# re-ovo/wgpu-path-tracing

Measured on AMD Instinct MI355X. Metric: Msamples/s (rays x bounces / s), higher is better.
Workload: dtype f32

## Files before the change

include/ptmi.h:

```cpp
#ifndef PTMI_H
#define PTMI_H

#include <stddef.h>
#include <stdint.h>
#include "ptmi_layout.h"

#ifdef __cplusplus
extern "C" {
#endif

#define PTMI_ABI_VERSION 4

enum {
    PTMI_OK = 0,
    PTMI_E_INVALID = -1,
    PTMI_E_NODEVICE = -2,
    PTMI_E_HIP = -3,
    PTMI_E_STATE = -4,
    PTMI_E_UNSUPPORTED = -5
};

enum { PTMI_ATLAS_RGBA16F = 1, PTMI_ATLAS_RGBA32F = 2 };
enum { PTMI_TRAVERSAL_AUTO = 0, PTMI_TRAVERSAL_GLOBAL = 1, PTMI_TRAVERSAL_LDS = 2, PTMI_TRAVERSAL_GLOBAL_EXACT = 3 };

// ... 16 lines not shown
    uint32_t tree_builder;
    uint32_t leaves;
    uint32_t leaf_tris;
    uint32_t reserved[1];
} ptmi_options;

typedef struct ptmi_stats {
    uint64_t paths;
    uint64_t segments;
    uint64_t shadow_rays;
    uint64_t dispatches;
    uint64_t frames;
    uint64_t segments_by_bounce[64];
    double   gpu_ms;
    double   extend_ms;
    uint64_t extend_launches;
    double   shade_ms;
    double   shadow_ms;
    uint32_t bvh_depth;
    uint32_t traversal_used;
    uint32_t frames_per_batch_used;
    uint32_t radiance_stride_bytes;
    uint64_t shadow_traced;
    uint64_t shade_launches, shadow_launches;
    double   raygen_ms, compact_ms, accumulate_ms;
    double   upload_ms;
    double   upload_tree_ms;
    double   upload_copy_ms;
    uint32_t leaves_used;
    uint32_t leaf_tris_used;
    uint32_t extend_variant, shadow_variant;
    uint64_t verify_failed;
    uint32_t tree_builder_used;
    uint32_t reserved_stats[1];
} ptmi_stats;

int ptmi_abi_version(void);
int ptmi_create(int device_ordinal, ptmi_ctx **out);
int ptmi_destroy(ptmi_ctx *ctx);
const char *ptmi_last_error(const ptmi_ctx *ctx);

int ptmi_upload_scene(ptmi_ctx *ctx,
                      const ptmi_triangle *triangles, uint32_t n_triangles,
                      const ptmi_material *materials, uint32_t n_materials,
                      const ptmi_bvh_node *bvh_nodes, uint32_t n_nodes,
                      const ptmi_light *lights, uint32_t n_lights);
int ptmi_upload_atlas(ptmi_ctx *ctx, const void *texels, uint32_t width, uint32_t height, int format);
int ptmi_resize(ptmi_ctx *ctx, uint32_t width, uint32_t height);
int ptmi_set_options(ptmi_ctx *ctx, const ptmi_options *opt);
int ptmi_get_options(const ptmi_ctx *ctx, ptmi_options *opt);

int ptmi_dispatch(ptmi_ctx *ctx, const ptmi_camera *camera, uint32_t n_frames);
int ptmi_synchronize(ptmi_ctx *ctx);
int ptmi_throttle(ptmi_ctx *ctx, uint32_t max_in_flight, uint32_t *in_flight);

int ptmi_read_output(ptmi_ctx *ctx, float *dst_rgba, size_t n_floats);
int ptmi_write_output(ptmi_ctx *ctx, const float *src_rgba, size_t n_floats);
void *ptmi_output_device_ptr(ptmi_ctx *ctx);
int ptmi_bind_output_device(ptmi_ctx *ctx, void *device_ptr, size_t bytes);
int ptmi_set_stream(ptmi_ctx *ctx, void *hip_stream);

enum { PTMI_AOV_ALBEDO = 1u, PTMI_AOV_NORMAL = 2u, PTMI_AOV_ID = 4u };
int ptmi_set_aovs(ptmi_ctx *ctx, uint32_t mask);
int ptmi_get_aovs(const ptmi_ctx *ctx, uint32_t *mask);
int ptmi_read_aov(ptmi_ctx *ctx, uint32_t which, void *dst, size_t n_bytes);
void *ptmi_aov_device_ptr(ptmi_ctx *ctx, uint32_t which);

// ... 99 lines not shown
```

wgpu-path-tracing_amd/csrc/pt_device.h:

```cpp
#pragma once
#include <hip/hip_runtime.h>
#include <stdint.h>
#include "ptmi_layout.h"
#include "ptmi.h"

#define PT_HD __host__ __device__ inline

#define PT_REF_LEAF      0x80000000u
#define PT_REF_NONE      0xFFFFFFFFu
#define PT_LEAF_MAX_TRIS 32u
#define PT_LEAF_OFF_BITS 26u
#define PT_LEAF_OFF_MASK ((1u << PT_LEAF_OFF_BITS) - 1u)

struct DevScene;
struct DevScene {
    const ptmi_triangle *tris;  uint32_t n_tris;
    const ptmi_material *mats;  uint32_t n_mats;
    const ptmi_light *lights;   uint32_t n_lights;
    const void *atlas;          uint32_t atlas_w, atlas_h, atlas_fmt;
    const float4 *wnodes;       uint32_t n_wnodes;
    const float4 *tripos;
    float root_min[3], root_max[3];
    uint32_t root_ref;
    const float4 *ref_wnodes;   uint32_t ref_root_ref, has_fast;
    const uint4 *qnodes;        const uint32_t *leaf_stream;
    float q_origin[3], q_scale[3];
    float tri_safe_dsum;
    uint32_t q_cached;
    uint32_t own, n_own_tris;
    const float4 *ref_tripos;
    const float4 *tri_leafbox;
    float ref_root_min[3], ref_root_max[3];
    float safe_origin;
    const float4 *wnodes16, *ref_wnodes16;
    uint32_t root_ref16, ref_root_ref16;
    const uint4 *qnodes16;
    unsigned long long *verify_stat;
    const DevScene *self;
};

struct rgb_sc { float x, y, z; };
struct DevPaths {
    float4 *O, *D; float2 *C; float *L; uint32_t l_stride = 3;
    __device__ __forceinline__ rgb_sc ldL(uint32_t p) const {
        if (l_stride == 4u) { const float4 v = reinterpret_cast<const float4 *>(L)[p]; return rgb_sc{v.x, v.y, v.z}; }
        return reinterpret_cast<const rgb_sc *>(L)[p];
    }
    __device__ __forceinline__ void stL(uint32_t p, float x, float y, float z) const {
        if (l_stride == 4u) reinterpret_cast<float4 *>(L)[p] = make_float4(x, y, z, 0.0f);
        else reinterpret_cast<rgb_sc *>(L)[p] = rgb_sc{x, y, z};
    }
};
struct DevShadow { float4 *SO, *SD; rgb_sc *SC; uint32_t cap; };

struct DevBand {
    uint32_t width, height, y0, y1, strip, parts, part, rows;
    PT_HD uint32_t row_of(uint32_t l) const {
        if (parts <= 1u) return y0 + l;
        return y0 + ((l / strip) * parts + part) * strip + l % strip;
    }
    PT_HD size_t frame_pixel(uint32_t pix) const { return (size_t)row_of(pix / width) * width + pix % width; }
};

PT_HD bool pt_plays_roulette(uint32_t bounce) { return bounce > 2u; }
inline uint32_t pt_repack_bounce() { uint32_t b = 0; while (!pt_plays_roulette(b)) b++; return b; }

struct ShadeParams {
    uint32_t bounce, max_bounces, do_mis;
    unsigned long long *stats;
    uint32_t emit_records;
    const uint32_t *pid;
};
// ... 141 lines not shown
```

wgpu-path-tracing_amd/csrc/ptmi_api.hip:

```cpp
#include "ptmi.h"
#include "pt_device.h"
#include "fast_tree.h"

#include <algorithm>
#include <chrono>
#include <cmath>
#include <cstdarg>
#include <cstdint>
#include <cstdio>
#include <cstring>
#include <deque>
#include <memory>
#include <string>
#include <typeinfo>
#include <utility>
#include <vector>

namespace {

thread_local std::string g_create_err;

enum SceneBuf {
    kTris, kMats, kLights,
    kRefWnodes, kRefTripos,
    kWnodes, kTripos,
    kQnodes, kLeafStream,
    kLeafbox,
    kWnodes16, kRefWnodes16, kQnodes16,
    kSceneBufs
};

enum FramePlane {
    kOut,
    kAovAlbedo, kAovNormal, kAovId,
    kMoments,
    kDnGuide, kDnGrad, kDnA, kDnB, kDnOut,
    kAdBallot, kAdList, kAdTileSums,
    kBlitF32, kBlitU8,
    kFramePlanes
};

enum LaneBuf {
    kPathO, kPathD, kPathC, kPathL,
    kHits,
    kShadow0, kShadowIdx0, kShadow1, kShadowIdx1,
    kTailO, kTailD, kTailC, kPid,
    kQueue0, kQueue1,
    kOcc,
    kAovRec,
    kLaneBufs
};

struct EventPair { hipEvent_t a, b; int kind; };
constexpr size_t kMaxPendingEvents = 4096;

}

struct Lane {
    size_t cap = 0;
    void *buf[kLaneBufs] = {};
    DevPaths paths{};
// ... 744 lines not shown

int ptmi_destroy(ptmi_ctx *c) {
    if (!c) return PTMI_E_INVALID;
    (void)hipSetDevice(c->device);
    (void)sync_all(c);
    drain_events(c);
    for (hipEvent_t e : c->in_flight) (void)hipEventDestroy(e);
    for (hipEvent_t e : c->event_pool) (void)hipEventDestroy(e);
    {
        Lane &ln = c->lane;
        free_batch(ln);
        dfree(ln.counts); dfree(ln.d_spill); dfree(ln.d_spill_side);
        for (hipEvent_t e : {ln.ev_ready, ln.ev_shadow[0], ln.ev_shadow[1]}) if (e) (void)hipEventDestroy(e);
        if (ln.side) (void)hipStreamDestroy(ln.side);
    }
    for (void *&p : c->buf) dfree(p);
    dfree(c->d_atlas);
    drop_planes(c, kAllPlanes);
    dfree(c->d_stats); dfree(c->d_scene); dfree(c->ad.ctl); dfree(c->ad.acc);
    if (c->own_stream) (void)hipStreamDestroy(c->own_stream);
    delete c;
    return PTMI_OK;
}

}

struct PtPrepared {
    Built b;
    uint32_t nt, nm, nl;
    double build_ms;
    bool take_device_buffers = false;
};

PtPrepared *pt_prepare_scene(ptmi_ctx *c, const ptmi_triangle *tris, uint32_t nt, const ptmi_material *mats, uint32_t nm,
                             const ptmi_bvh_node *nodes, uint32_t nn, const ptmi_light *lights, uint32_t nl, int *rc_out) {
    auto bad = [&](int rc) -> PtPrepared * { *rc_out = rc; return nullptr; };
    if (!c) return bad(PTMI_E_INVALID);
    if ((nt && !tris) || (nm && !mats) || (nn && !nodes) || (nl && !lights))
        return bad(fail(c, PTMI_E_INVALID, "NULL blob with a non-zero count"));
    if (hipSetDevice(c->device) != hipSuccess) return bad(fail(c, PTMI_E_HIP, "hipSetDevice(%d) failed", c->device));
    for (uint32_t i = 0; i < nl; i++) {
        if (lights[i].light_type > PTMI_LIGHT_POINT)
            return bad(fail(c, PTMI_E_INVALID, "light %u has unknown type %u", i, lights[i].light_type));
        if (lights[i].light_type == PTMI_LIGHT_EMISSIVE && lights[i].triangle_index >= nt)
            return bad(fail(c, PTMI_E_INVALID, "emissive light %u references triangle %u of %u", i, lights[i].triangle_index, nt));
    }
    const auto t_start = std::chrono::steady_clock::now();
    PtPrepared *p = new PtPrepared();
    int rc = build_image(c->opt, c->stream, c->device, tris, nt, nodes, nn, p->b, c->err);
    if (rc) { delete p; return bad(rc); }
    if (!p->b.buf[kTris].present) p->b.view(kTris, tris, (size_t)nt * sizeof(ptmi_triangle));
    p->b.view(kMats, mats, (size_t)nm * sizeof(ptmi_material));
    p->b.view(kLights, lights, (size_t)nl * sizeof(ptmi_light));
    p->nt = nt; p->nm = nm; p->nl = nl;
    p->build_ms = std::chrono::duration<double, std::milli>(std::chrono::steady_clock::now() - t_start).count();
    *rc_out = PTMI_OK;
    return p;
}
void pt_free_prepared(PtPrepared *p) { delete p; }

int pt_install_scene(ptmi_ctx *c, PtPrepared *prep) {
    if (!c || !prep) return PTMI_E_INVALID;
    HIP_TRY(c, hipSetDevice(c->device));
    using clk = std::chrono::steady_clock;
    auto ms_since = [](clk::time_point t0) { return std::chrono::duration<double, std::milli>(clk::now() - t0).count(); };
    const auto t_start = clk::now();
    Built &b = prep->b;
    const auto t_copy = clk::now();
    void *n[kSceneBufs] = {};
    hipError_t e = hipSuccess;
    for (int k = 0; k < kSceneBufs && e == hipSuccess; k++) {
        HeldBuf &h = b.buf[k];
        if (!h.present) continue;
        if (h.dev && prep->take_device_buffers && h.device == c->device) { n[k] = h.dev; h.dev = nullptr; continue; }
        e = hipMalloc(&n[k], h.bytes ? h.bytes : 16);
        if (e != hipSuccess) break;
        if (h.dev) e = h.device == c->device ? hipMemcpy(n[k], h.dev, h.bytes, hipMemcpyDeviceToDevice)
                                             : hipMemcpyPeer(n[k], c->device, h.dev, h.device, h.bytes);
        else e = h.bytes ? hipMemcpy(n[k], h.host, h.bytes, hipMemcpyHostToDevice) : hipMemset(n[k], 0, 16);
    }
    if (e != hipSuccess) {
        for (void *&p : n) dfree(p);
        return fail(c, PTMI_E_HIP, "scene upload failed: %s (the previous scene, if any, is still in place)", hipGetErrorString(e));
    }
    HIP_TRY(c, sync_all(c));
    for (int k = 0; k < kSceneBufs; k++) { dfree(c->buf[k]); c->buf[k] = n[k]; }
    void *const *d = c->buf;
    const ptmi_image_info &h = b.img;
    const bool own = h.leaves_used == 2u;
    DevScene &s = c->sc;
    s.tris = static_cast<const ptmi_triangle *>(d[kTris]); s.n_tris = prep->nt;
    s.mats = static_cast<const ptmi_material *>(d[kMats]); s.n_mats = prep->nm;
    s.lights = static_cast<const ptmi_light *>(d[kLights]); s.n_lights = prep->nl;
    s.ref_wnodes = static_cast<const float4 *>(d[kRefWnodes]); s.ref_root_ref = b.ref_root_ref; s.has_fast = d[kWnodes] ? 1u : 0u;
    s.wnodes = static_cast<const float4 *>(walked(d, kWnodes));
    s.n_wnodes = h.n_wnodes;
    s.tripos = static_cast<const float4 *>(walked(d, kTripos));
    s.ref_tripos = static_cast<const float4 *>(d[kRefTripos]);
    s.qnodes = static_cast<const uint4 *>(d[kQnodes]); s.leaf_stream = static_cast<const uint32_t *>(d[kLeafStream]);
    for (int k = 0; k < 3; k++) { s.q_origin[k] = h.q_origin[k]; s.q_scale[k] = h.q_scale[k]; }
    s.q_cached = b.q_top;
    s.tri_safe_dsum = b.tri_safe_dsum;
    for (int k = 0; k < 3; k++) {
        s.ref_root_min[k] = b.ref_root_min[k]; s.ref_root_max[k] = b.ref_root_max[k];
        s.root_min[k] = h.root_min[k]; s.root_max[k] = h.root_max[k];
    }
    s.root_ref = h.root_ref;
    s.own = own ? 1u : 0u;
    s.n_own_tris = own ? h.n_tris : 0u;
    s.tri_leafbox = static_cast<const float4 *>(d[kLeafbox]);
    s.wnodes16 = static_cast<const float4 *>(d[kWnodes16]); s.ref_wnodes16 = static_cast<const float4 *>(d[kRefWnodes16]);
    s.qnodes16 = static_cast<const uint4 *>(d[kQnodes16]);
    s.root_ref16 = b.root_ref16; s.ref_root_ref16 = b.ref_root_ref16;
    s.safe_origin = h.safe_origin;
    s.verify_stat = c->d_stats + 4;
    s.self = c->d_scene;
    HIP_TRY(c, hipMemcpy(c->d_scene, &c->sc, sizeof(DevScene), hipMemcpyHostToDevice));
    c->img = h;
    c->have_scene = true;
    c->st.leaves_used = h.leaves_used;
    c->st.leaf_tris_used = h.max_leaf_tris;
    c->st.tree_builder_used = b.tree_builder_used;
    c->st.upload_copy_ms = ms_since(t_copy);
    c->st.upload_tree_ms = b.tree_ms;
    c->st.upload_ms = prep->build_ms + ms_since(t_start);
    return PTMI_OK;
}

extern "C" {

int ptmi_upload_scene(ptmi_ctx *c, const ptmi_triangle *tris, uint32_t nt, const ptmi_material *mats, uint32_t nm,
                      const ptmi_bvh_node *nodes, uint32_t nn, const ptmi_light *lights, uint32_t nl) {
    int rc = PTMI_OK;
    PtPrepared *p = pt_prepare_scene(c, tris, nt, mats, nm, nodes, nn, lights, nl, &rc);
    if (!p) return rc;
    p->take_device_buffers = true;
    rc = pt_install_scene(c, p);
    pt_free_prepared(p);
    return rc;
}

}

int pt_atlas_bytes(uint32_t w, uint32_t h, int fmt, size_t *bytes, char *why, size_t why_len) {
    *bytes = 0;
    if (fmt != PTMI_ATLAS_RGBA16F && fmt != PTMI_ATLAS_RGBA32F) {
        snprintf(why, why_len, "unknown atlas format %d", fmt);
        return PTMI_E_INVALID;
    }
// ... 100 lines not shown
    const uint64_t npix = (uint64_t)band.rows * band.width;
    uint32_t F = c->opt.frames_per_batch;
    const bool auto_F = F == 0;
    Lane &ln = c->lane;
    if (auto_F) {
        F = (uint32_t)std::max<uint64_t>(1, std::min<uint64_t>(64, (128ull << 20) / npix));
        size_t free_b = 0, total_b = 0;
        if (hipMemGetInfo(&free_b, &total_b) == hipSuccess) {
            const uint64_t held = (uint64_t)ln.cap * bytes_per_path(ln.aov != nullptr);
            const uint64_t room = (uint64_t)((double)(free_b + held) * 0.9);
            F = (uint32_t)std::max<uint64_t>(1, std::min<uint64_t>(F, room / (npix * bytes_per_path(c->aov_mask != 0))));
        }
    }
    F = std::min(F, n_frames);
    const bool nee = c->opt.do_mis && c->sc.n_lights > 0;
    const bool side = nee && c->opt.overlap != 0;
    if (npix * F > 0xFFFFFF00ull) return fail(c, PTMI_E_UNSUPPORTED, "batch of %llu paths exceeds 2^32", (unsigned long long)(npix * F));
    const TraverseConfig cfg0 = traverse_config(c, true), cfg_shadow0 = traverse_config(c, false);
    if (c->opt.traversal == PTMI_TRAVERSAL_LDS && pt_variant(cfg0.variant).where != PT_LDS_ALL)
        return fail(c, PTMI_E_UNSUPPORTED, "scene needs %zu B of LDS plus the stack; it does not fit in %zu B", lds_scene_bytes(c), kLdsMax);
    for (;;) {
        rc = ensure_capacity(c, ln, (size_t)(npix * F));
        if (rc == PTMI_OK) break;
        if (!auto_F || !c->alloc_oom || F <= 1) return rc;
        F = (F + 1) / 2;
    }
    if (cfg0.wants_spill && !ln.d_spill) HIP_TRY(c, hipMalloc(&ln.d_spill, pt_spill_bytes(c->n_cu * 8)));
    if (cfg_shadow0.wants_spill && !ln.d_spill_side) HIP_TRY(c, hipMalloc(&ln.d_spill_side, pt_spill_bytes(c->n_cu * 8)));
    c->st.traversal_used = pt_variant(cfg0.variant).where == PT_FROM_MEMORY ? PTMI_TRAVERSAL_GLOBAL : PTMI_TRAVERSAL_LDS;
    c->st.extend_variant = pt_variant_code(cfg0);
    c->st.shadow_variant = pt_variant_code(cfg_shadow0);
    c->st.frames_per_batch_used = F;
    c->st.radiance_stride_bytes = (walks_memory_quantised(cfg0) || walks_memory_quantised(cfg_shadow0)) ? 16u : 12u;
    const int blocks = c->n_cu * 8;
#ifndef PT_SHADE_WGS_PER_CU
#define PT_SHADE_WGS_PER_CU 16
#endif
    const int shade_blocks = c->n_cu * PT_SHADE_WGS_PER_CU;
    const uint32_t maxb = c->opt.max_bounces;
    const bool t1 = c->opt.timing >= 1, t2 = c->opt.timing >= 2, t3 = c->opt.timing >= 3;
    {
        Timed td(c, 0, t1);
        const hipStream_t ms = c->stream;
        const hipStream_t ss = side ? ln.side : ms;
        const int tiles = (int)(ln.cap / pt_compact_tile_slots() + 1);
        TraverseConfig cfg = cfg0, cfg_shadow = cfg_shadow0;
        cfg.spill = ln.d_spill; cfg_shadow.spill = side ? ln.d_spill_side : ln.d_spill;
        if (cfg_shadow.wants_spill && !cfg_shadow.spill) cfg_shadow.spill = ln.d_spill_side;
        ln.paths.l_stride = c->st.radiance_stride_bytes / 4u;
        const DevPaths bp = ln.paths;
        const uint32_t rb = PT_REPACK ? pt_repack_bounce() : 0xFFFFFFFEu;
        DevPaths tp = ln.tail;
        tp.L = bp.L; tp.l_stride = bp.l_stride;
        float4 *const aov_rec = c->aov_mask ? ln.aov : nullptr;
        float4 *const mom = plane_as<float4>(c, kMoments);
        if (ap && cam->frame_index == 0u) { pt_launch_adaptive_restart(ms, blocks, band, mom); c->ad_rounds = 0; }
        auto batch = [&](uint32_t frame0, uint32_t fb) -> int {
            const DevPixels px = ap ? DevPixels{band, 0u, c->ad.list, &c->ad.ctl[1], mom, c->ad.acc}
                                    : DevPixels{band, frame0, nullptr, nullptr, nullptr, nullptr};
            { Timed t(c, 4, t3, ms); pt_launch_raygen(ms, blocks, *cam, px, fb, bp, &ln.counts[0]); }
            int cur = 0;
            for (uint32_t b = 0; b < maxb; b++) {
                const bool tail = b > rb;
                const uint32_t *q = b == 0 || b == rb + 1 ? nullptr : ln.queue[cur];
                const DevPaths sp = tail ? tp : bp;
                const int par = side ? (int)(b & 1u) : 0;
// ... 572 lines not shown
```

wgpu-path-tracing_amd/csrc/shade.hip:

```cpp
#include "pt_device.h"
#include "pt_math.h"

namespace {

struct HitInfo {
    v3 position; float t;
    v3 normal;
    v3 albedo;
    float roughness, metallic, transmission, ior;
    v3 emission; float emissive_strength;
    bool is_front;
};

PT_DEV v3 ld3(const float *p) { return mk3(p[0], p[1], p[2]); }

PT_DEV v4 atlas_load(const DevScene &sc, uint32_t x, uint32_t y) {
    v4 r; r.x = r.y = r.z = r.w = 0.0f;
    if (sc.atlas_fmt == 0u || x >= sc.atlas_w || y >= sc.atlas_h) return r;
    size_t idx = ((size_t)y * sc.atlas_w + x);
    if (sc.atlas_fmt == 1u) {
        const uint2 raw = reinterpret_cast<const uint2 *>(sc.atlas)[idx];
        union { uint32_t u; _Float16 h[2]; } a, b;
        a.u = raw.x; b.u = raw.y;
        r.x = (float)a.h[0]; r.y = (float)a.h[1]; r.z = (float)b.h[0]; r.w = (float)b.h[1];
    } else {
        const float4 t = reinterpret_cast<const float4 *>(sc.atlas)[idx];
        r.x = t.x; r.y = t.y; r.z = t.z; r.w = t.w;
    }
    return r;
}

PT_DEV v4 texture_color(const DevScene &sc, const ptmi_atlas_rect &tx, float uvx, float uvy, v4 fallback) {
    if (tx.w == 0u || tx.h == 0u) return fallback;
    float fx = uvx - __builtin_truncf(uvx);
    float fy = uvy - __builtin_truncf(uvy);
    float ax = (float)tx.x + fx * (float)tx.w;
    float ay = (float)tx.y + fy * (float)tx.h;
    return atlas_load(sc, f2u(ax), f2u(ay));
}

PT_DEV HitInfo make_hitinfo(const DevScene &sc, v3 ro, v3 rd, float t, uint32_t tri) {
    HitInfo hi;
    const ptmi_triangle &T = sc.tris[tri];
    const v3 tv0 = ld3(T.v0), tv1 = ld3(T.v1), tv2 = ld3(T.v2);
    const v3 tn0 = ld3(T.n0), tn1 = ld3(T.n1), tn2 = ld3(T.n2);
    const float u0x = T.uv0[0], u0y = T.uv0[1], u1x = T.uv1[0], u1y = T.uv1[1], u2x = T.uv2[0], u2y = T.uv2[1];
    const uint32_t mi = T.material_index;
    v3 v0 = tv0;
    v3 e1 = sub3(tv1, v0), e2 = sub3(tv2, v0);
    float u, v;
    (void)tri_test(v0, e1, e2, ro, rd, u, v);
    hi.t = t;
    hi.position = madd3(rd, t, ro);
    float w = 1.0f - u - v;
    v3 geo_n = normalize3(cross3(e1, e2));
    v3 n_i = normalize3(lincomb3(tn0, w, tn1, u, tn2, v));
    float uvx = fma1(u2x, v, fma1(u1x, u, u0x * w));
    float uvy = fma1(u2y, v, fma1(u1y, u, u0y * w));
    hi.is_front = dot3(geo_n, rd) < 0.0f;
    ptmi_material m;
    if (mi < sc.n_mats) m = sc.mats[mi];
    else __builtin_memset(&m, 0, sizeof m);
    v4 one; one.x = one.y = one.z = one.w = 1.0f;
    v4 alb = texture_color(sc, m.albedo_map, uvx, uvy, one);
    hi.albedo = mk3(alb.x * m.base_color[0], alb.y * m.base_color[1], alb.z * m.base_color[2]);
    v4 pbr = texture_color(sc, m.pbr_map, uvx, uvy, one);
    hi.metallic = pbr.z * m.metallic;
    hi.roughness = max1(pbr.y * m.roughness, 0.04f);
    hi.transmission = m.transmission;
    hi.ior = m.ior;
    v4 em = texture_color(sc, m.emissive_map, uvx, uvy, one);
    hi.emission = mk3(em.x * m.emission[0], em.y * m.emission[1], em.z * m.emission[2]);
    hi.emissive_strength = m.emissive_strength;
    v4 flat; flat.x = 0.5f; flat.y = 0.5f; flat.z = 1.0f; flat.w = 1.0f;
    v4 nm = texture_color(sc, m.normal_map, uvx, uvy, flat);
    if (nm.x != 0.5f || nm.y != 0.5f || nm.z != 1.0f) {
        float du1x = u1x - u0x, du1y = u1y - u0y;
        float du2x = u2x - u0x, du2y = u2y - u0y;
        float rr = rcp1(fma1(du1x, du2y, -(du1y * du2x)));
        v3 tg = mk3(fma1(e1.x, du2y, -(e2.x * du1y)) * rr, fma1(e1.y, du2y, -(e2.y * du1y)) * rr,
                    fma1(e1.z, du2y, -(e2.z * du1y)) * rr);
        tg = normalize3(tg);
        v3 N = n_i;
        v3 Tn = normalize3(madd3(N, -dot3(N, tg), tg));
        v3 Bn = normalize3(cross3(N, Tn));
        float tx = nm.x * 2.0f - 1.0f, ty = nm.y * 2.0f - 1.0f, tz = nm.z * 2.0f - 1.0f;
        hi.normal = normalize3(lincomb3(Tn, tx, Bn, ty, N, tz));
    } else {
        hi.normal = n_i;
    }
    return hi;
}

PT_DEV float distribution_ggx(v3 N, v3 H, float roughness) {
    float a = roughness * roughness;
// ... 72 lines not shown
    float ndh = max1(dot3(normal, H), 0.0f);
    float vdh = max1(dot3(V, H), 0.0f);
    v3 F0 = mk3(mix1(0.04f, h.albedo.x, h.metallic), mix1(0.04f, h.albedo.y, h.metallic),
                mix1(0.04f, h.albedo.z, h.metallic));
    v3 F = fresnel_schlick(vdh, F0);
    float G = geometry_smith(normal, V, L, h.roughness);
    float D = distribution_ggx(normal, H, h.roughness);
    float one_m_tr = 1.0f - h.transmission;
    v3 kD = mk3((1.0f - F.x) * one_m_tr, (1.0f - F.y) * one_m_tr, (1.0f - F.z) * one_m_tr);
    v3 diffuse = vdiv3(mul3(kD, h.albedo), PT_PI);
    v3 specular = vdiv3(scale3(scale3(F, G), D), max1(4.0f * ndv * ndl, PT_EPS));
    v3 bsdf = mk3(0.0f, 0.0f, 0.0f);
    float pdf = 0.0f;
    if (h.transmission > 0.0f) {
        float eta = front ? rcp1(h.ior) : h.ior;
        float cos_t = dot3(normal, V);
        float Ft = reflectance(__builtin_fabsf(cos_t), eta);
        bsdf = scale3(h.albedo, 1.0f - Ft);
        pdf = (1.0f - h.metallic) * h.transmission;
    } else {
        bsdf = scale3(add3(diffuse, specular), ndl);
        float diffuse_p = (1.0f - h.metallic) * (1.0f - h.transmission);
        float specular_p = h.metallic;
        float diffuse_pdf = ndl / PT_PI;
        float specular_pdf = D * ndh / (4.0f * vdh);
        pdf = diffuse_p * diffuse_pdf + specular_p * specular_pdf;
    }
    v4 r; r.x = bsdf.x; r.y = bsdf.y; r.z = bsdf.z; r.w = max1(pdf, PT_EPS);
    return r;
}

struct LightSample { v3 intensity; v3 wi; float pdf; float dist; bool traced; };

PT_DEV LightSample sample_light(const DevScene &sc, uint32_t &rng, v3 hit_pos) {
    LightSample ls;
    ls.intensity = mk3(0.0f, 0.0f, 0.0f); ls.wi = mk3(0.0f, 0.0f, 0.0f); ls.pdf = 0.0f; ls.dist = -1.0f; ls.traced = false;
    const uint32_t nl = sc.n_lights;
    const ptmi_light lt = sc.lights[rng_int(rng, 0u, nl - 1u)];
    const float inv_n = rcp1((float)nl);
    if (lt.light_type == PTMI_LIGHT_DIRECTIONAL) {
        ls.wi = normalize3(neg3(ld3(lt.position)));
        ls.intensity = scale3(ld3(lt.color), lt.intensity);
        ls.pdf = inv_n * 1000.0f;
        ls.dist = -1.0f;
        ls.traced = true;
    } else if (lt.light_type == PTMI_LIGHT_POINT) {
        v3 to_l = sub3(ld3(lt.position), hit_pos);
        float dist = length3(to_l);
        if (dist > 100.0f) return ls;
        ls.wi = vdiv3(to_l, dist);
        float att = rcp1(dist * dist);
        ls.intensity = scale3(scale3(ld3(lt.color), lt.intensity), att);
        ls.pdf = inv_n * 10000.0f;
        ls.dist = dist;
        ls.traced = true;
    } else if (lt.light_type == PTMI_LIGHT_EMISSIVE) {
        ptmi_triangle T;
        if (lt.triangle_index < sc.n_tris) T = sc.tris[lt.triangle_index];
        else __builtin_memset(&T, 0, sizeof T);
        float r1 = rng_f(rng), r2 = rng_f(rng);
        float sq = sqrt1(r1);
        float u = 1.0f - sq;
        float v = r2 * sq;
        float w = 1.0f - u - v;
        v3 lp = lincomb3(ld3(T.v0), w, ld3(T.v1), u, ld3(T.v2), v);
        v3 n = normalize3(lincomb3(ld3(T.n0), w, ld3(T.n1), u, ld3(T.n2), v));
        v3 to_l = sub3(lp, hit_pos);
        float dist = length3(to_l);
        v3 wi = vdiv3(to_l, dist);
        v3 e1 = sub3(ld3(T.v1), ld3(T.v0)), e2 = sub3(ld3(T.v2), ld3(T.v0));
        float area = length3(cross3(e1, e2)) * 0.5f;
        float cos_t = __builtin_fabsf(dot3(n, neg3(wi)));
        ls.pdf = (inv_n * rcp1(area)) * (dist * dist / max1(cos_t, PT_EPS));
        ls.intensity = scale3(ld3(lt.color), lt.intensity);
        ls.wi = wi;
        ls.dist = dist;
        ls.traced = true;
    }
    return ls;
}

constexpr int SBLOCK = 256;
#ifndef PT_SHADE_WAVES
#define PT_SHADE_WAVES 0
#endif
#if PT_SHADE_WAVES > 0
#define PT_SHADE_ATTR __attribute__((amdgpu_waves_per_eu(PT_SHADE_WAVES)))
#else
#define PT_SHADE_ATTR
#endif

template <bool AOV>
__global__ __launch_bounds__(SBLOCK) PT_SHADE_ATTR void k_shade(DevScene sc, DevPaths P, const uint32_t *__restrict__ queue,
                                                  const uint32_t *__restrict__ count_ptr,
                                                  const float2 *__restrict__ hits, DevShadow S,
                                                  uint64_t *__restrict__ alive_mask,
                                                  uint64_t *__restrict__ shadow_mask, ShadeParams sp,
                                                  float4 *__restrict__ aov) {
    const uint32_t count = *count_ptr;
    const uint32_t lane = threadIdx.x & 63u;
    uint32_t n_skipped = 0, n_emitted = 0;
    for (uint32_t base = blockIdx.x * SBLOCK; base < count; base += gridDim.x * SBLOCK) {
        const uint32_t i = base + threadIdx.x;
        bool alive = false, shadow = false, skipped = false, emitted = false;
        float4 rec_o = make_float4(0.0f, 0.0f, 0.0f, -2.0f), rec_d = make_float4(0.0f, 0.0f, 0.0f, 0.0f);
        rgb_sc rec_c{0.0f, 0.0f, 0.0f};
        if (i < count) {
            const uint32_t q = queue ? queue[i] : i;
            const float2 h2 = ld_stream(&hits[i]);
            if (!(h2.x < 0.0f)) {
                const float4 o4 = ld_stream(&P.O[q]), d4 = ld_stream(&P.D[q]);
                const uint32_t p = sp.pid ? sp.pid[q] : q;
                uint32_t rng = __float_as_uint(o4.w);
                const v3 ro = xyz(o4), rd = xyz(d4);
                v3 thr = mk3(1.0f, 1.0f, 1.0f);
                if (sp.bounce != 0u) { const float2 c2 = ld_stream(&P.C[q]); thr = mk3(d4.w, c2.x, c2.y); }
                const HitInfo hit = make_hitinfo(sc, ro, rd, h2.x, __float_as_uint(h2.y));
                if (AOV) {
                    st_stream(&aov[2 * (size_t)i], make_float4(hit.albedo.x, hit.albedo.y, hit.albedo.z, hit.t));
                    st_stream(&aov[2 * (size_t)i + 1], make_float4(hit.normal.x, hit.normal.y, hit.normal.z, h2.y));
                }
                if (hit.emission.x > 0.0f || hit.emission.y > 0.0f || hit.emission.z > 0.0f) {
                    float att = rcp1(1.0f + hit.t * hit.t);
                    float k = hit.emissive_strength;
                    const v3 e = mk3(thr.x * hit.emission.x * k * att, thr.y * hit.emission.y * k * att, thr.z * hit.emission.z * k * att);
                    if (sp.emit_records) {
                        rec_d.w = __uint_as_float(p);
                        rec_c = rgb_sc{e.x, e.y, e.z};
                        shadow = true; emitted = true;
                    } else {
                        const rgb_sc l = P.ldL(p);
                        P.stL(p, l.x + e.x, l.y + e.y, l.z + e.z);
                    }
                } else {
                    if (sp.do_mis && sc.n_lights > 0u && hit.transmission == 0.0f && hit.is_front) {
                        LightSample ls = sample_light(sc, rng, hit.position);
                        if (ls.pdf > 0.0f) {
                            v3 V = neg3(normalize3(rd));
                            v4 ev = eval_bsdf(hit, hit.normal, V, ls.wi, hit.is_front);
                            float wmis = power_heuristic(1.0f, ls.pdf, 1.0f, ev.w);
                            v3 direct = vdiv3(scale3(mul3(ls.intensity, mk3(ev.x, ev.y, ev.z)), wmis),
                                              max1(ls.pdf, PT_EPS));
                            v3 contrib = mul3(thr, direct);
                            if ((contrib.x != 0.0f) | (contrib.y != 0.0f) | (contrib.z != 0.0f)) {
                                v3 so = madd3(ls.wi, PT_EPS, hit.position);
                                rec_o = make_float4(so.x, so.y, so.z, ls.dist);
                                rec_d = make_float4(ls.wi.x, ls.wi.y, ls.wi.z, __uint_as_float(p));
                                rec_c = rgb_sc{contrib.x, contrib.y, contrib.z};
                                shadow = true;
                            } else {
                                skipped = true;
                            }
                        } else if (ls.traced) {
                            skipped = true;
                        }
                    }
                    v3 dir = sample_bsdf(rng, hit, rd, hit.is_front);
                    v4 ev = eval_bsdf(hit, hit.normal, neg3(normalize3(rd)), dir, hit.is_front);
                    if (!(ev.w <= 0.0f)) {
                        v3 no = madd3(dir, PT_EPS, hit.position);
                        v3 nd = normalize3(dir);
                        thr = mul3(thr, vdiv3(mk3(ev.x, ev.y, ev.z), max1(ev.w, PT_EPS)));
                        alive = true;
                        if (pt_plays_roulette(sp.bounce)) {
                            float pr = max1(max1(thr.x, thr.y), thr.z);
                            if (rng_f(rng) > pr) alive = false;
                            else thr = vdiv3(thr, pr);
                        }
                        if (alive && sp.bounce + 1u < sp.max_bounces) {
// ... 18 lines not shown
                        shadow = true; emitted = true;
                    } else {
                        const rgb_sc l = P.ldL(p);
                        P.stL(p, l.x + e.x, l.y + e.y, l.z + e.z);
                    }
                }
            }
        }
        const uint64_t am = __ballot(alive), sm = __ballot(shadow), zm = __ballot(skipped), em = __ballot(emitted);
        if (shadow) {
            const uint32_t r = (i & ~63u) + (uint32_t)__popcll(sm & ((1ull << lane) - 1ull));
            st_stream(&S.SO[r], rec_o);
            st_stream(&S.SD[r], rec_d);
            S.SC[r] = rec_c;
        }
        if (lane == 0u && i < count) {
            alive_mask[i >> 6] = am;
            shadow_mask[i >> 6] = sm;
            n_skipped += (uint32_t)__popcll(zm);
            n_emitted += (uint32_t)__popcll(em);
        }
    }
    if (n_skipped) atomicAdd(&sp.stats[1], (unsigned long long)n_skipped);
    if (n_emitted) atomicAdd(&sp.stats[3], (unsigned long long)n_emitted);
}

}

#ifdef PT_SHADE_FAST
#define PT_LAUNCH_SHADE pt_launch_shade_fast
#else
#define PT_LAUNCH_SHADE pt_launch_shade
#endif
void PT_LAUNCH_SHADE(hipStream_t s, int blocks, const DevScene &sc, DevPaths p, const uint32_t *queue,
                     const uint32_t *count, const float2 *hits, DevShadow sh, uint64_t *alive_mask,
                     uint64_t *shadow_mask, ShadeParams sp, float4 *aov) {
    if (aov)
        hipLaunchKernelGGL(k_shade<true>, dim3(blocks), dim3(SBLOCK), 0, s, sc, p, queue, count, hits, sh, alive_mask,
                           shadow_mask, sp, aov);
    else
        hipLaunchKernelGGL(k_shade<false>, dim3(blocks), dim3(SBLOCK), 0, s, sc, p, queue, count, hits, sh, alive_mask,
                           shadow_mask, sp, aov);
}

#ifndef PT_SHADE_FAST
namespace {
__global__ void k_hit_uv(uint32_t n, DevScene sc, DevPaths P, const float2 *__restrict__ hits, float2 *__restrict__ uv) {
    const uint32_t i = blockIdx.x * blockDim.x + threadIdx.x;
    if (i >= n) return;
    const float2 h = hits[i];
    float u = 0.0f, v = 0.0f;
    if (!(h.x < 0.0f)) {
        const ptmi_triangle &T = sc.tris[__float_as_uint(h.y)];
        const v3 v0 = ld3(T.v0);
        (void)tri_test(v0, sub3(ld3(T.v1), v0), sub3(ld3(T.v2), v0), xyz(P.O[i]), xyz(P.D[i]), u, v);
    }
    uv[i] = make_float2(u, v);
}
}
void pt_launch_hit_uv(hipStream_t s, uint32_t n, const DevScene &sc, DevPaths p, const float2 *hits, float2 *uv) {
    hipLaunchKernelGGL(k_hit_uv, dim3((n + 255) / 256), dim3(256), 0, s, n, sc, p, hits, uv);
}
#endif
```

wgpu-path-tracing_amd/ptmi/native.py:

```python
import ctypes
import functools
import os
import types

import numpy as np

from . import layout

_LIB_DIR = os.path.join(os.path.dirname(os.path.dirname(os.path.abspath(__file__))), "lib")
LIB_PATH = os.environ.get("PTMI_LIB") or os.path.join(_LIB_DIR, "libptmi.so")

TRAVERSAL_AUTO, TRAVERSAL_GLOBAL, TRAVERSAL_LDS, TRAVERSAL_GLOBAL_EXACT = 0, 1, 2, 3
ATLAS_RGBA16F, ATLAS_RGBA32F = 1, 2

EXPORTS = [
    "ptmi_abi_version", "ptmi_create", "ptmi_destroy", "ptmi_last_error", "ptmi_upload_scene",
    "ptmi_upload_atlas", "ptmi_resize", "ptmi_set_options", "ptmi_get_options", "ptmi_dispatch",
    "ptmi_synchronize", "ptmi_read_output", "ptmi_write_output", "ptmi_output_device_ptr",
    "ptmi_bind_output_device", "ptmi_set_stream", "ptmi_blit", "ptmi_get_stats", "ptmi_reset_stats",
    "ptmi_debug_raygen", "ptmi_debug_intersect", "ptmi_debug_occluded", "ptmi_debug_math", "ptmi_debug_exact_math", "ptmi_get_size",
    "ptmi_debug_image_stats", "ptmi_debug_build_image", "ptmi_debug_read_image", "ptmi_throttle", "ptmi_multi_throttle",
    "ptmi_multi_create", "ptmi_multi_destroy", "ptmi_multi_last_error", "ptmi_multi_count", "ptmi_multi_context",
    "ptmi_multi_upload_scene", "ptmi_multi_upload_atlas", "ptmi_multi_resize", "ptmi_multi_set_options", "ptmi_multi_get_options",
    "ptmi_multi_dispatch", "ptmi_multi_gather", "ptmi_multi_synchronize", "ptmi_multi_read_output", "ptmi_multi_write_output",
# ... 28 lines not shown

class DenoiseParams(ctypes.Structure):
    _fields_ = [("iterations", ctypes.c_uint32), ("demodulate", ctypes.c_uint32), ("phi_color", ctypes.c_float),
                ("phi_normal", ctypes.c_float), ("phi_depth", ctypes.c_float), ("reserved", ctypes.c_uint32 * 3)]


class AdaptiveParams(ctypes.Structure):
    _fields_ = [("threshold", ctypes.c_float), ("floor", ctypes.c_float), ("min_frames", ctypes.c_uint32),
                ("max_frames", ctypes.c_uint32), ("step", ctypes.c_uint32), ("neighbourhood", ctypes.c_uint32),
                ("reserved", ctypes.c_uint32 * 2)]


class AdaptiveStatus(ctypes.Structure):
    _fields_ = [("active", ctypes.c_uint64), ("samples", ctypes.c_uint64), ("min_count", ctypes.c_uint32),
                ("max_count", ctypes.c_uint32), ("rounds", ctypes.c_uint32), ("reserved", ctypes.c_uint32)]

    def as_dict(self):
        return {n: int(getattr(self, n)) for n, _ in self._fields_ if n != "reserved"}


class Stats(ctypes.Structure):
    _fields_ = [("paths", ctypes.c_uint64), ("segments", ctypes.c_uint64), ("shadow_rays", ctypes.c_uint64),
                ("dispatches", ctypes.c_uint64), ("frames", ctypes.c_uint64),
                ("segments_by_bounce", ctypes.c_uint64 * 64),
                ("gpu_ms", ctypes.c_double), ("extend_ms", ctypes.c_double), ("extend_launches", ctypes.c_uint64),
                ("shade_ms", ctypes.c_double), ("shadow_ms", ctypes.c_double),
                ("bvh_depth", ctypes.c_uint32), ("traversal_used", ctypes.c_uint32),
                ("frames_per_batch_used", ctypes.c_uint32), ("radiance_stride_bytes", ctypes.c_uint32),
                ("shadow_traced", ctypes.c_uint64), ("shade_launches", ctypes.c_uint64), ("shadow_launches", ctypes.c_uint64),
                ("raygen_ms", ctypes.c_double), ("compact_ms", ctypes.c_double), ("accumulate_ms", ctypes.c_double),
                ("upload_ms", ctypes.c_double), ("upload_tree_ms", ctypes.c_double), ("upload_copy_ms", ctypes.c_double),
                ("leaves_used", ctypes.c_uint32), ("leaf_tris_used", ctypes.c_uint32),
                ("extend_variant", ctypes.c_uint32), ("shadow_variant", ctypes.c_uint32), ("verify_failed", ctypes.c_uint64),
                ("tree_builder_used", ctypes.c_uint32), ("reserved_stats", ctypes.c_uint32 * 1)]

    def as_dict(self):
        d = {k: getattr(self, k) for k, _ in self._fields_ if k not in ("segments_by_bounce", "reserved_stats")}
        d["segments_by_bounce"] = [int(v) for v in self.segments_by_bounce if v]
        return d


_SHARED = {
    "destroy": [], "last_error": [], "synchronize": [], "reset_stats": [], "resize": [ctypes.c_uint32, ctypes.c_uint32],
    "upload_scene": [ctypes.c_void_p, ctypes.c_uint32] * 4,
    "upload_atlas": [ctypes.c_void_p, ctypes.c_uint32, ctypes.c_uint32, ctypes.c_int],
    "set_options": [ctypes.c_void_p], "get_options": [ctypes.c_void_p], "dispatch": [ctypes.c_void_p, ctypes.c_uint32],
    "throttle": [ctypes.c_uint32, ctypes.POINTER(ctypes.c_uint32)], "read_output": [ctypes.c_void_p, ctypes.c_size_t],
    "write_output": [ctypes.c_void_p, ctypes.c_size_t], "blit": [ctypes.c_void_p, ctypes.c_size_t] * 2,
    "get_stats": [ctypes.c_void_p],
}
_lib = None


def load():
    global _lib
    if _lib is None:
        if not os.path.exists(LIB_PATH):
            raise PtmiError(-2, f"{LIB_PATH} is missing: build it with `python __graft_entry__.py build`")
        L = ctypes.CDLL(LIB_PATH)
        for name in EXPORTS:
            getattr(L, name)
        if L.ptmi_abi_version() != ABI_VERSION:
            raise PtmiError(-1, f"{LIB_PATH} has ABI {L.ptmi_abi_version()}, this binding expects {ABI_VERSION}: rebuild it")
        vp, u32, sz = ctypes.c_void_p, ctypes.c_uint32, ctypes.c_size_t
        for prefix in ("ptmi_", "ptmi_multi_"):
            for name, args in _SHARED.items():
                getattr(L, prefix + name).argtypes = [vp] + args
        L.ptmi_last_error.restype = L.ptmi_multi_last_error.restype = ctypes.c_char_p
        L.ptmi_create.argtypes = [ctypes.c_int, vp]
        L.ptmi_output_device_ptr.restype = vp
# ... 357 lines not shown
```

Baseline: 11060.

## Stage material and light tables in LDS for the shade kernel

Builds a packed host-side table of materials, lights and emissive light triangles, uploads it, and has each shade workgroup copy it into shared memory at kernel start. Material, light and light-triangle lookups then read LDS instead of global memory, chosen at compile time through a STAGE template and picked at launch by a 16 KB budget. This is meant to cut scattered global loads during shading, at the cost of a per-block preload, a barrier, and LDS use that may lower occupancy.

```diff
diff --git a/include/ptmi.h b/include/ptmi.h
--- a/include/ptmi.h
+++ b/include/ptmi.h
@@ -72,7 +72,7 @@
     uint32_t extend_variant, shadow_variant;
     uint64_t verify_failed;
     uint32_t tree_builder_used;
-    uint32_t reserved_stats[1];
+    uint32_t shade_tables;
 } ptmi_stats;
 
 int ptmi_abi_version(void);
diff --git a/wgpu-path-tracing_amd/csrc/pt_device.h b/wgpu-path-tracing_amd/csrc/pt_device.h
--- a/wgpu-path-tracing_amd/csrc/pt_device.h
+++ b/wgpu-path-tracing_amd/csrc/pt_device.h
@@ -37,7 +37,19 @@
     const uint4 *qnodes16;
     unsigned long long *verify_stat;
     const DevScene *self;
-};
+    const float4 *shade_tab;
+};
+
+#define PT_SHADE_LDS_BUDGET 16384u
+enum { PT_STAGE_MATS = 1, PT_STAGE_LIGHTS = 2 };
+PT_HD size_t pt_tab_mats_q(uint32_t n_mats) { return ((size_t)n_mats + 1u) * 8u; }
+PT_HD size_t pt_tab_lights_q(uint32_t n_lights) { return (size_t)n_lights * 11u; }
+PT_HD int pt_shade_stage(uint32_t n_mats, uint32_t n_lights) {
+    const size_t m = pt_tab_mats_q(n_mats) * 16u, l = pt_tab_lights_q(n_lights) * 16u;
+    if (m + l <= PT_SHADE_LDS_BUDGET) return PT_STAGE_MATS | (n_lights ? PT_STAGE_LIGHTS : 0);
+    if (m <= PT_SHADE_LDS_BUDGET) return PT_STAGE_MATS;
+    return l <= PT_SHADE_LDS_BUDGET && n_lights ? PT_STAGE_LIGHTS : 0;
+}
 
 struct rgb_sc { float x, y, z; };
 struct DevPaths {
diff --git a/wgpu-path-tracing_amd/csrc/ptmi_api.hip b/wgpu-path-tracing_amd/csrc/ptmi_api.hip
--- a/wgpu-path-tracing_amd/csrc/ptmi_api.hip
+++ b/wgpu-path-tracing_amd/csrc/ptmi_api.hip
@@ -27,6 +27,7 @@
     kQnodes, kLeafStream,
     kLeafbox,
     kWnodes16, kRefWnodes16, kQnodes16,
+    kShadeTab,
     kSceneBufs
 };
 
@@ -837,6 +838,20 @@
     bool take_device_buffers = false;
 };
 
+static std::vector<float4> shade_tables(const ptmi_triangle *tris, uint32_t nt, const ptmi_material *mats, uint32_t nm,
+                                        const ptmi_light *lights, uint32_t nl) {
+    std::vector<float4> tab(pt_tab_mats_q(nm) + pt_tab_lights_q(nl), make_float4(0.0f, 0.0f, 0.0f, 0.0f));
+    char *at = reinterpret_cast<char *>(tab.data());
+    if (nm) std::memcpy(at, mats, (size_t)nm * sizeof(ptmi_material));
+    at += pt_tab_mats_q(nm) * sizeof(float4);
+    if (nl) std::memcpy(at, lights, (size_t)nl * sizeof(ptmi_light));
+    at += (size_t)nl * sizeof(ptmi_light);
+    for (uint32_t i = 0; i < nl; i++)
+        if (lights[i].light_type == PTMI_LIGHT_EMISSIVE && lights[i].triangle_index < nt)
+            std::memcpy(at + (size_t)i * sizeof(ptmi_triangle), &tris[lights[i].triangle_index], sizeof(ptmi_triangle));
+    return tab;
+}
+
 PtPrepared *pt_prepare_scene(ptmi_ctx *c, const ptmi_triangle *tris, uint32_t nt, const ptmi_material *mats, uint32_t nm,
                              const ptmi_bvh_node *nodes, uint32_t nn, const ptmi_light *lights, uint32_t nl, int *rc_out) {
     auto bad = [&](int rc) -> PtPrepared * { *rc_out = rc; return nullptr; };
@@ -857,6 +872,7 @@
     if (!p->b.buf[kTris].present) p->b.view(kTris, tris, (size_t)nt * sizeof(ptmi_triangle));
     p->b.view(kMats, mats, (size_t)nm * sizeof(ptmi_material));
     p->b.view(kLights, lights, (size_t)nl * sizeof(ptmi_light));
+    p->b.hold(kShadeTab, shade_tables(tris, nt, mats, nm, lights, nl));
     p->nt = nt; p->nm = nm; p->nl = nl;
     p->build_ms = std::chrono::duration<double, std::milli>(std::chrono::steady_clock::now() - t_start).count();
     *rc_out = PTMI_OK;
@@ -920,6 +936,7 @@
     s.safe_origin = h.safe_origin;
     s.verify_stat = c->d_stats + 4;
     s.self = c->d_scene;
+    s.shade_tab = static_cast<const float4 *>(d[kShadeTab]);
     HIP_TRY(c, hipMemcpy(c->d_scene, &c->sc, sizeof(DevScene), hipMemcpyHostToDevice));
     c->img = h;
     c->have_scene = true;
@@ -1086,6 +1103,7 @@
     c->st.shadow_variant = pt_variant_code(cfg_shadow0);
     c->st.frames_per_batch_used = F;
     c->st.radiance_stride_bytes = (walks_memory_quantised(cfg0) || walks_memory_quantised(cfg_shadow0)) ? 16u : 12u;
+    c->st.shade_tables = PT_SHADE_LDS_BUDGET | ((uint32_t)pt_shade_stage(c->sc.n_mats, c->sc.n_lights) << 28);
     const int blocks = c->n_cu * 8;
 #ifndef PT_SHADE_WGS_PER_CU
 #define PT_SHADE_WGS_PER_CU 16
diff --git a/wgpu-path-tracing_amd/csrc/shade.hip b/wgpu-path-tracing_amd/csrc/shade.hip
--- a/wgpu-path-tracing_amd/csrc/shade.hip
+++ b/wgpu-path-tracing_amd/csrc/shade.hip
@@ -13,6 +13,36 @@
 };
 
 PT_DEV v3 ld3(const float *p) { return mk3(p[0], p[1], p[2]); }
+
+typedef float f4v __attribute__((ext_vector_type(4)));
+typedef const __attribute__((address_space(3))) f4v *lds_f4p;
+template <class R, int Q> PT_DEV R lds_record(lds_f4p p) {
+    static_assert(sizeof(R) == Q * 16, "a record of Q quads");
+    R r;
+    __builtin_memcpy(&r, p, sizeof r);
+    return r;
+}
+template <int STAGE> struct ShadeTabs {
+    lds_f4p mats, lights, ltris;
+    PT_DEV ptmi_material material(const DevScene &sc, uint32_t mi) const {
+        if (STAGE & PT_STAGE_MATS) return lds_record<ptmi_material, 8>(mats + 8u * min(mi, sc.n_mats));
+        ptmi_material m;
+        if (mi < sc.n_mats) m = sc.mats[mi];
+        else __builtin_memset(&m, 0, sizeof m);
+        return m;
+    }
+    PT_DEV ptmi_light light(const DevScene &sc, uint32_t li) const {
+        if (STAGE & PT_STAGE_LIGHTS) return lds_record<ptmi_light, 3>(lights + 3u * li);
+        return sc.lights[li];
+    }
+    PT_DEV ptmi_triangle light_triangle(const DevScene &sc, uint32_t li, uint32_t triangle_index) const {
+        if (STAGE & PT_STAGE_LIGHTS) return lds_record<ptmi_triangle, 8>(ltris + 8u * li);
+        ptmi_triangle T;
+        if (triangle_index < sc.n_tris) T = sc.tris[triangle_index];
+        else __builtin_memset(&T, 0, sizeof T);
+        return T;
+    }
+};
 
 PT_DEV v4 atlas_load(const DevScene &sc, uint32_t x, uint32_t y) {
     v4 r; r.x = r.y = r.z = r.w = 0.0f;
@@ -39,7 +69,8 @@
     return atlas_load(sc, f2u(ax), f2u(ay));
 }
 
-PT_DEV HitInfo make_hitinfo(const DevScene &sc, v3 ro, v3 rd, float t, uint32_t tri) {
+template <int STAGE>
+PT_DEV HitInfo make_hitinfo(const DevScene &sc, const ShadeTabs<STAGE> &tabs, v3 ro, v3 rd, float t, uint32_t tri) {
     HitInfo hi;
     const ptmi_triangle &T = sc.tris[tri];
     const v3 tv0 = ld3(T.v0), tv1 = ld3(T.v1), tv2 = ld3(T.v2);
@@ -58,9 +89,7 @@
     float uvx = fma1(u2x, v, fma1(u1x, u, u0x * w));
     float uvy = fma1(u2y, v, fma1(u1y, u, u0y * w));
     hi.is_front = dot3(geo_n, rd) < 0.0f;
-    ptmi_material m;
-    if (mi < sc.n_mats) m = sc.mats[mi];
-    else __builtin_memset(&m, 0, sizeof m);
+    const ptmi_material m = tabs.material(sc, mi);
     v4 one; one.x = one.y = one.z = one.w = 1.0f;
     v4 alb = texture_color(sc, m.albedo_map, uvx, uvy, one);
     hi.albedo = mk3(alb.x * m.base_color[0], alb.y * m.base_color[1], alb.z * m.base_color[2]);
@@ -199,11 +228,13 @@
 
 struct LightSample { v3 intensity; v3 wi; float pdf; float dist; bool traced; };
 
-PT_DEV LightSample sample_light(const DevScene &sc, uint32_t &rng, v3 hit_pos) {
+template <int STAGE>
+PT_DEV LightSample sample_light(const DevScene &sc, const ShadeTabs<STAGE> &tabs, uint32_t &rng, v3 hit_pos) {
     LightSample ls;
     ls.intensity = mk3(0.0f, 0.0f, 0.0f); ls.wi = mk3(0.0f, 0.0f, 0.0f); ls.pdf = 0.0f; ls.dist = -1.0f; ls.traced = false;
     const uint32_t nl = sc.n_lights;
-    const ptmi_light lt = sc.lights[rng_int(rng, 0u, nl - 1u)];
+    const uint32_t li = rng_int(rng, 0u, nl - 1u);
+    const ptmi_light lt = tabs.light(sc, li);
     const float inv_n = rcp1((float)nl);
     if (lt.light_type == PTMI_LIGHT_DIRECTIONAL) {
         ls.wi = normalize3(neg3(ld3(lt.position)));
@@ -222,9 +253,7 @@
         ls.dist = dist;
         ls.traced = true;
     } else if (lt.light_type == PTMI_LIGHT_EMISSIVE) {
-        ptmi_triangle T;
-        if (lt.triangle_index < sc.n_tris) T = sc.tris[lt.triangle_index];
-        else __builtin_memset(&T, 0, sizeof T);
+        const ptmi_triangle T = tabs.light_triangle(sc, li, lt.triangle_index);
         float r1 = rng_f(rng), r2 = rng_f(rng);
         float sq = sqrt1(r1);
         float u = 1.0f - sq;
@@ -257,15 +286,25 @@
 #define PT_SHADE_ATTR
 #endif
 
-template <bool AOV>
+template <bool AOV, int STAGE>
 __global__ __launch_bounds__(SBLOCK) PT_SHADE_ATTR void k_shade(DevScene sc, DevPaths P, const uint32_t *__restrict__ queue,
                                                   const uint32_t *__restrict__ count_ptr,
                                                   const float2 *__restrict__ hits, DevShadow S,
                                                   uint64_t *__restrict__ alive_mask,
                                                   uint64_t *__restrict__ shadow_mask, ShadeParams sp,
                                                   float4 *__restrict__ aov) {
+    extern __shared__ float4 smem[];
     const uint32_t count = *count_ptr;
     const uint32_t lane = threadIdx.x & 63u;
+    const uint32_t mats_q = (STAGE & PT_STAGE_MATS) ? (uint32_t)pt_tab_mats_q(sc.n_mats) : 0u;
+    const uint32_t lights_q = (STAGE & PT_STAGE_LIGHTS) ? (uint32_t)pt_tab_lights_q(sc.n_lights) : 0u;
+    if (STAGE) {
+        const float4 *src = sc.shade_tab + ((STAGE & PT_STAGE_MATS) ? 0u : pt_tab_mats_q(sc.n_mats));
+        for (uint32_t k = threadIdx.x; k < mats_q + lights_q; k += SBLOCK) smem[k] = src[k];
+        __syncthreads();
+    }
+    const lds_f4p lds_lights = (lds_f4p)smem + mats_q;
+    const ShadeTabs<STAGE> tabs{(lds_f4p)smem, lds_lights, lds_lights + 3u * sc.n_lights};
     uint32_t n_skipped = 0, n_emitted = 0;
     for (uint32_t base = blockIdx.x * SBLOCK; base < count; base += gridDim.x * SBLOCK) {
         const uint32_t i = base + threadIdx.x;
@@ -282,7 +321,7 @@
                 const v3 ro = xyz(o4), rd = xyz(d4);
                 v3 thr = mk3(1.0f, 1.0f, 1.0f);
                 if (sp.bounce != 0u) { const float2 c2 = ld_stream(&P.C[q]); thr = mk3(d4.w, c2.x, c2.y); }
-                const HitInfo hit = make_hitinfo(sc, ro, rd, h2.x, __float_as_uint(h2.y));
+                const HitInfo hit = make_hitinfo(sc, tabs, ro, rd, h2.x, __float_as_uint(h2.y));
                 if (AOV) {
                     st_stream(&aov[2 * (size_t)i], make_float4(hit.albedo.x, hit.albedo.y, hit.albedo.z, hit.t));
                     st_stream(&aov[2 * (size_t)i + 1], make_float4(hit.normal.x, hit.normal.y, hit.normal.z, h2.y));
@@ -301,7 +340,7 @@
                     }
                 } else {
                     if (sp.do_mis && sc.n_lights > 0u && hit.transmission == 0.0f && hit.is_front) {
-                        LightSample ls = sample_light(sc, rng, hit.position);
+                        LightSample ls = sample_light(sc, tabs, rng, hit.position);
                         if (ls.pdf > 0.0f) {
                             v3 V = neg3(normalize3(rd));
                             v4 ev = eval_bsdf(hit, hit.normal, V, ls.wi, hit.is_front);
@@ -386,15 +425,27 @@
 #else
 #define PT_LAUNCH_SHADE pt_launch_shade
 #endif
+namespace {
+template <bool AOV, int STAGE>
+void launch_shade(hipStream_t s, int blocks, const DevScene &sc, DevPaths p, const uint32_t *queue, const uint32_t *count,
+                  const float2 *hits, DevShadow sh, uint64_t *alive_mask, uint64_t *shadow_mask, ShadeParams sp, float4 *aov) {
+    const size_t lds = (((STAGE & PT_STAGE_MATS) ? pt_tab_mats_q(sc.n_mats) : 0) + ((STAGE & PT_STAGE_LIGHTS) ? pt_tab_lights_q(sc.n_lights) : 0)) * 16;
+    hipLaunchKernelGGL((k_shade<AOV, STAGE>), dim3(blocks), dim3(SBLOCK), lds, s, sc, p, queue, count, hits, sh, alive_mask,
+                       shadow_mask, sp, aov);
+}
+}
 void PT_LAUNCH_SHADE(hipStream_t s, int blocks, const DevScene &sc, DevPaths p, const uint32_t *queue,
                      const uint32_t *count, const float2 *hits, DevShadow sh, uint64_t *alive_mask,
                      uint64_t *shadow_mask, ShadeParams sp, float4 *aov) {
-    if (aov)
-        hipLaunchKernelGGL(k_shade<true>, dim3(blocks), dim3(SBLOCK), 0, s, sc, p, queue, count, hits, sh, alive_mask,
-                           shadow_mask, sp, aov);
-    else
-        hipLaunchKernelGGL(k_shade<false>, dim3(blocks), dim3(SBLOCK), 0, s, sc, p, queue, count, hits, sh, alive_mask,
-                           shadow_mask, sp, aov);
+#define PT_SHADE_CASE(STAGE)                                                                                              \
+    case STAGE:                                                                                                           \
+        (aov ? launch_shade<true, STAGE> : launch_shade<false, STAGE>)(s, blocks, sc, p, queue, count, hits, sh, alive_mask, \
+                                                                       shadow_mask, sp, aov);                             \
+        break;
+    switch (pt_shade_stage(sc.n_mats, sc.n_lights)) {
+        PT_SHADE_CASE(0) PT_SHADE_CASE(PT_STAGE_MATS) PT_SHADE_CASE(PT_STAGE_LIGHTS) PT_SHADE_CASE(PT_STAGE_MATS | PT_STAGE_LIGHTS)
+    }
+#undef PT_SHADE_CASE
 }
 
 #ifndef PT_SHADE_FAST
diff --git a/wgpu-path-tracing_amd/ptmi/native.py b/wgpu-path-tracing_amd/ptmi/native.py
--- a/wgpu-path-tracing_amd/ptmi/native.py
+++ b/wgpu-path-tracing_amd/ptmi/native.py
@@ -84,10 +84,10 @@
                 ("upload_ms", ctypes.c_double), ("upload_tree_ms", ctypes.c_double), ("upload_copy_ms", ctypes.c_double),
                 ("leaves_used", ctypes.c_uint32), ("leaf_tris_used", ctypes.c_uint32),
                 ("extend_variant", ctypes.c_uint32), ("shadow_variant", ctypes.c_uint32), ("verify_failed", ctypes.c_uint64),
-                ("tree_builder_used", ctypes.c_uint32), ("reserved_stats", ctypes.c_uint32 * 1)]
+                ("tree_builder_used", ctypes.c_uint32), ("shade_tables", ctypes.c_uint32)]
 
     def as_dict(self):
-        d = {k: getattr(self, k) for k, _ in self._fields_ if k not in ("segments_by_bounce", "reserved_stats")}
+        d = {k: getattr(self, k) for k, _ in self._fields_ if k != "segments_by_bounce"}
         d["segments_by_bounce"] = [int(v) for v in self.segments_by_bounce if v]
         return d
 
```

Result: faster. 11650, median of 6 (+5.3%).
